# bharath5673/StrongSORT-YOLO

Measured on AMD Instinct MI355X. Metric: tracked frames/sec (whole node), 1280x720@30det, higher is better.
Workload: dtype f32 association / f64 Kalman+LSAP (f16 detector convs, fp32 ReID network on own v_mfma_f32 kernels)

## Files before the change

include/strongsort_hip.h:

```cpp
#ifndef STRONGSORT_HIP_H
#define STRONGSORT_HIP_H
#include <stdint.h>

#ifdef __cplusplus
extern "C" {
#endif

#define SS_OK 0
#define SS_ERR_INVALID (-1)
#define SS_ERR_CAPACITY (-2)
#define SS_ERR_HIP (-3)
#define SS_ERR_INFEASIBLE (-4)

#define SS_FEAT_DIM 512
#define SS_MAX_TRACKS 256
#define SS_MAX_DETS 128
#define SS_OUT_COLS 8

typedef struct ss_ctx ss_ctx;

typedef struct ss_config {
    double max_dist;
    double max_iou_distance;
    double mc_lambda;
// ... 165 lines not shown
                      void* d_out2, int c0, int cn);
int ss_op_bottleneck_f16(void* stream, const void* d_x, const void* d_w1, const void* d_b1, const void* d_w2, const void* d_b2,
                         int B, int H, int W, int C, int add, void* d_out, int out_ld, void* d_out2);
typedef struct ss_conv_desc {
    const void* x; const void* w; const void* bias; void* out;
    int B, H, W, Cin, N, ksize, stride, act;
} ss_conv_desc;
int ss_op_conv_group_f16(void* stream, int n, const ss_conv_desc* descs);
int ss_op_head_f16(void* stream, const void* d_x, const void* const* d_w1, const void* const* d_b1, const void* const* d_w2,
                   const void* const* d_b2, const void* const* d_w3, const void* const* d_b3, void* const* d_out, const int* nout,
                   int B, int H, int W, int Cin, int tile16);
int ss_op_v8_decode_f16(void* stream, const void* const* d_box, const void* const* d_cls, const void* const* d_box_bias,
                        const void* const* d_cls_bias, const int* H, const int* W, const int* strides, int B, int nc,
                        float* d_pred);
int ss_op_v8_decode_ext_f16(void* stream, const void* const* d_box, const void* const* d_cls, const void* const* d_box_bias,
                            const void* const* d_cls_bias, const void* const* d_ext, int n_ext, int ext_ld, int ext_mode,
                            const int* H, const int* W, const int* strides, int B, int nc, int cls_ld, float* d_pred);
int ss_op_dwconv3x3_f16(void* stream, const void* d_x, const void* d_w9 , const void* d_bias, void* d_y,
                        int N, int H, int W, int C, int act);
int ss_op_lightconv_f16(void* stream, const void* d_x, const void* d_w1, const void* d_w9, const void* d_bias,
                        void* d_y, int N, int H, int W, int C);
int ss_op_conv0_f16(void* stream, const void* d_x, const void* d_w_prep, const void* d_bias, void* d_y, int B, int H, int W, int Cout,
                    int act);
int ss_op_set_valid_images(void* stream, const int* d_n, int batch);
int ss_op_set_option(const char* name, int value);
int ss_op_osnet_stem_f16(void* stream, const void* d_x, const void* d_w_prep, const void* d_bias, void* d_y, int N, int H,
                         int W, const void* d_w1 , const void* d_b1, void* d_y1);
int ss_op_osnet_streams_bands(int N, int H, int W, int C);
int ss_op_osnet_streams_f16(void* stream, const void* d_x, const void* d_w1, const void* d_dwtab,
                            void* const* d_ys, float* d_psum, int N, int H, int W, int C);
long long ss_op_dwtab_bytes(int layers, int C);
int ss_op_dwtab_f16(void* stream, const void* d_w9, const void* d_bias, int layers, int C, void* d_out);
int ss_op_gate_apply_f16(void* stream, const void* const* d_xs, int T, const void* d_w1, const void* d_b1,
                         const void* d_w2, const void* d_b2, const float* d_sums, int parts, float scale, void* d_out,
                         int N, int HW, int C, int Cr);
int ss_op_osnet_tail_f16(void* stream, const void* const* d_ys, const float* d_psum, int parts, float scale, const void* d_gw1,
                         const void* d_gb1, const void* d_gw2, const void* d_gb2, int Cr, float* d_gates_ws ,
                         const void* d_w3, const void* d_b3, const void* d_idn, int C1, const void* d_wd, const void* d_bd,
                         void* d_out, const void* d_w4, const void* d_b4, void* d_out2, int pool, int N, int H, int W, int MID,
                         int C2, int N2);
int ss_op_upcat_f16(void* stream, const void* d_lo, const void* d_hi, void* d_out, int B, int h, int w, int C1, int C2, int lo_first);
int ss_op_sppf_pools_f16(void* stream, const void* d_x, void* d_out, int B, int H, int W, int C);
int ss_op_psa_attention_f16(void* stream, const void* d_qkv, const void* d_pe, void* d_out, int B, int N, int heads, float scale);
int ss_op_osnet_head_f16(void* stream, const void* d_x, const void* d_w, const void* d_bias, void* d_out, int N, int HW, int C, int F);
int ss_op_avgpool2_f16(void* stream, const void* d_x, void* d_y, int N, int H, int W, int C);
int ss_op_maxpool_f16(void* stream, const void* d_x, void* d_y, int N, int H, int W, int C, int k, int stride, int pad);
// ... 48 lines not shown
```

strongsort_yolo_amd/csrc/ss_front.hip:

```cpp
#include <hip/hip_fp16.h>
#include "ss_common.h"

__device__ inline void ss_axis(int d, float scale, int n_src, int& i0, int& i1, float& frac)
{
    float t = (float)d + 0.5f;
    float s = t * scale;
    float f = s - 0.5f;
    int i = (int)floorf(f);
    float fr = f - (float)i;
    if (i < 0) { i = 0; fr = 0.0f; }
    if (i >= n_src - 1) { i = n_src - 1; fr = 0.0f; i1 = i; } else i1 = i + 1;
    i0 = i; frac = fr;
}

__device__ inline float ss_bilerp_u8(float p00, float p01, float p10, float p11, float fx, float fy)
{
    float a = fmaf(fx, p01 - p00, p00);
    float b = fmaf(fx, p11 - p10, p10);
    float v = fmaf(fy, b - a, a);
    float q = floorf(v + 0.5f);
    return fminf(fmaxf(q, 0.0f), 255.0f);
}

template <typename T> __device__ inline T ss_cvt(float v);
template <> __device__ inline float ss_cvt<float>(float v) { return v; }
template <> __device__ inline __half ss_cvt<__half>(float v) { return __float2half(v); }
template <typename T> struct ss_is_u8 { static constexpr bool value = false; };
template <> struct ss_is_u8<uint8_t> { static constexpr bool value = true; };

template <typename T, int HWC>
__global__ __launch_bounds__(256) void k_letterbox(const uint8_t* __restrict__ src, long long src_batch_stride,
                                                   int H, int W, int stride, T* __restrict__ dst, int out_h,
                                                   int out_w, int new_h, int new_w, int pad_top, int pad_left,
                                                   float padv)
{
    const int x = blockIdx.x * blockDim.x + threadIdx.x;
    const int y = blockIdx.y;
    if (x >= out_w) return;
    const size_t plane = (size_t)out_h * out_w;
    src += (size_t)blockIdx.z * src_batch_stride;
    dst += (size_t)blockIdx.z * 3 * plane;
    const size_t o = HWC ? ((size_t)y * out_w + x) * 3 : (size_t)y * out_w + x;
    const size_t cs = HWC ? 1 : plane;
    const int ry = y - pad_top, rx = x - pad_left;
    if (ry < 0 || ry >= new_h || rx < 0 || rx >= new_w) {
        T p = ss_cvt<T>(padv);
        dst[o] = p; dst[cs + o] = p; dst[2 * cs + o] = p;
        return;
    }
    const float sx = (float)W / (float)new_w, sy = (float)H / (float)new_h;
    int y0, y1, x0, x1; float fy, fx;
    ss_axis(ry, sy, H, y0, y1, fy);
    ss_axis(rx, sx, W, x0, x1, fx);
    const uint8_t* r0 = src + (size_t)y0 * stride;
    const uint8_t* r1 = src + (size_t)y1 * stride;
#pragma unroll
    for (int c = 0; c < 3; ++c) {
        const int sc = 2 - c;
        float p00 = r0[x0 * 3 + sc], p01 = r0[x1 * 3 + sc], p10 = r1[x0 * 3 + sc], p11 = r1[x1 * 3 + sc];
        dst[c * cs + o] = ss_cvt<T>(ss_bilerp_u8(p00, p01, p10, p11, fx, fy) / 255.0f);
    }
}

void ss_launch_letterbox(const uint8_t* src, int batch, long long src_batch_stride, int h, int w, int stride, void* dst,
                         int flags, int out_h, int out_w, int new_h, int new_w, int pad_top, int pad_left,
                         int pad_value, hipStream_t st)
{
    if (batch <= 0) return;
    dim3 grid((out_w + 255) / 256, out_h, batch), block(256);
    float padv = (float)pad_value / 255.0f;
#define SS_LB(T, L) hipLaunchKernelGGL((k_letterbox<T, L>), grid, block, 0, st, src, src_batch_stride, h, w, stride, \
                                       (T*)dst, out_h, out_w, new_h, new_w, pad_top, pad_left, padv)
    switch (flags & 3) {
    case 0: SS_LB(float, 0); break;
    case 1: SS_LB(__half, 0); break;
    case 2: SS_LB(float, 1); break;
    default: SS_LB(__half, 1); break;
    }
#undef SS_LB
}

template <typename T, int HWC>
__global__ __launch_bounds__(128) void k_crop(const uint8_t* __restrict__ src, long long src_batch_stride, int H, int W,
// ... 714 lines not shown
```

strongsort_yolo_amd/csrc/ss_ops.hip:

```cpp
#include <hip/hip_fp16.h>
#include <hip/hip_runtime.h>
#include <stdint.h>
#include <stdlib.h>
#include <string>
#include "../../include/strongsort_hip.h"

struct NvEntry { void* stream; const int* n; int batch; };
static thread_local NvEntry g_nv[8] = {};
static inline const int* nv_for(void* stream, long long batch)
{
    for (const NvEntry& e : g_nv) if (e.n && e.stream == stream && e.batch == batch) return e.n;
    return nullptr;
}
static inline int nv_batch(void* stream)
{
    for (const NvEntry& e : g_nv) if (e.n && e.stream == stream) return e.batch;
    return 0;
}

static int g_opt_pw_epilogue = 1, g_opt_pw_splitk = 1, g_opt_osnet_chains = 1;

typedef _Float16 h8 __attribute__((ext_vector_type(8)));
typedef _Float16 h4 __attribute__((ext_vector_type(4)));
typedef float f4 __attribute__((ext_vector_type(4)));

__device__ inline float act_apply(float v, int act)
{
    if (act == 1) return v > 0.f ? v : 0.f;
// ... 941 lines not shown
        const h4 b1 = *reinterpret_cast<const h4*>(b1c + 4 * q);
#pragma unroll
        for (int pt = 0; pt < 2; ++pt) {
            const h8 bv = kv ? *reinterpret_cast<const h8*>(In + (size_t)(r * 32 + pt * 16 + n) * 24 + 8 * q) : z8;
            const h4 v0 = { bv[0], bv[1], bv[2], bv[3] }, v1 = { bv[4], bv[5], bv[6], bv[7] };
            f4 d = { 0.f, 0.f, 0.f, 0.f };
            d = __builtin_amdgcn_mfma_f32_16x16x16f16(a0, v0, d, 0, 0, 0);
            d = __builtin_amdgcn_mfma_f32_16x16x16f16(a1, v1, d, 0, 0, 0);
            h4 o;
#pragma unroll
            for (int j = 0; j < 4; ++j) {
                const float f = (float)(_Float16)d[j] + (float)b1[j];
                o[j] = (_Float16)(f > 0.f ? f : 0.f);
            }
            *reinterpret_cast<h4*>(y1 + (((size_t)img * OHp + j0 + r) * 32 + pt * 16 + n) * 16 + 4 * q) = o;
        }
    }
}

#define C0_PITCH 400
#define C0_ROWS 8

template <int COUT>
__global__ __launch_bounds__(256) void k_conv0(const __half* __restrict__ x, const __half* __restrict__ wp, const __half* __restrict__ bias,
                                              __half* __restrict__ y, int H, int W, int act)
{
    constexpr int MT = COUT / 16, IN_ROWS = 2 * C0_ROWS + 1, CH = C0_PITCH / 8;
    __shared__ __attribute__((aligned(16))) _Float16 In[IN_ROWS * C0_PITCH];
    const int tid = threadIdx.x, lane = tid & 63, r = tid >> 6, q = lane >> 4, n = lane & 15;
    const int OH = (H - 1) / 2 + 1, OW = W / 2;
    const int c0 = blockIdx.x * 64, oy0 = blockIdx.y * C0_ROWS, b = blockIdx.z;
    const h8 z8 = { 0, 0, 0, 0, 0, 0, 0, 0 };
    const __half* xi = x + (size_t)b * H * W * 3;
    const int row_halfs = W * 3, f0 = 6 * c0 - 8;
    for (int i = tid; i < IN_ROWS * CH; i += 256) {
        const int rr = i / CH, ch = i - rr * CH, gr = 2 * oy0 - 1 + rr, f = f0 + ch * 8;
        *reinterpret_cast<h8*>(In + rr * C0_PITCH + ch * 8) =
            (gr >= 0 && gr < H && f >= 0 && f + 8 <= row_halfs) ? *reinterpret_cast<const h8*>(xi + (size_t)gr * row_halfs + f) : z8;
    }
    h4 a[MT][3], bb[MT];
#pragma unroll
    for (int mt = 0; mt < MT; ++mt) {
#pragma unroll
        for (int ky = 0; ky < 3; ++ky) a[mt][ky] = *reinterpret_cast<const h4*>(wp + ((size_t)(r * 3 + ky) * COUT + mt * 16 + n) * 16 + 4 * q);
        bb[mt] = *reinterpret_cast<const h4*>(bias + mt * 16 + 4 * q);
    }
    __syncthreads();
    const _Float16* bp = In + 8 * (3 * n + (6 * r + 5) / 8) + 4 * q;
    const int c = c0 + 4 * n + r;
#pragma unroll 2
    for (int cr = 0; cr < C0_ROWS; ++cr) {
        const int oy = oy0 + cr;
        if (oy >= OH) break;
        h4 bv[3];
#pragma unroll
        for (int ky = 0; ky < 3; ++ky) bv[ky] = *reinterpret_cast<const h4*>(bp + (2 * cr + ky) * C0_PITCH);
#pragma unroll
        for (int mt = 0; mt < MT; ++mt) {
            f4 d = { 0.f, 0.f, 0.f, 0.f };
#pragma unroll
            for (int ky = 0; ky < 3; ++ky) d = __builtin_amdgcn_mfma_f32_16x16x16f16(a[mt][ky], bv[ky], d, 0, 0, 0);
            h4 o;
#pragma unroll
            for (int j = 0; j < 4; ++j) o[j] = (_Float16)act_apply((float)(_Float16)d[j] + (float)bb[mt][j], act);
            if (c < OW) *reinterpret_cast<h4*>(y + (((size_t)b * OH + oy) * OW + c) * COUT + mt * 16 + 4 * q) = o;
        }
    }
}

#define LC_TH 16

template <int C>
struct DwDiag {
    static constexpr int MT = (C + 15) / 16;
    h8 A1[MT][3], A2[MT][3];
    f4 bf[MT];
    __device__ __forceinline__ void init(const __half* __restrict__ w9l, const __half* __restrict__ biasl, int q, int n)
    {
#pragma unroll
        for (int mt = 0; mt < MT; ++mt) {
            const int c = mt * 16 + n, c4 = mt * 16 + 4 * q;
            const bool on = c < C && (n >> 2) == q;
#pragma unroll
            for (int ky = 0; ky < 3; ++ky) {
                const _Float16 w0 = on ? (_Float16)__half2float(w9l[(ky * 3 + 0) * C + c]) : (_Float16)0.f;
                const _Float16 w1 = on ? (_Float16)__half2float(w9l[(ky * 3 + 1) * C + c]) : (_Float16)0.f;
                const _Float16 w2 = on ? (_Float16)__half2float(w9l[(ky * 3 + 2) * C + c]) : (_Float16)0.f;
                h8 a1 = { 0, 0, 0, 0, 0, 0, 0, 0 }, a2 = { 0, 0, 0, 0, 0, 0, 0, 0 };
#pragma unroll
                for (int j = 0; j < 4; ++j) {
// ... 1535 lines not shown

extern "C" int ss_op_sppf_pools_f16(void* stream, const void* x, void* out, int B, int H, int W, int C)
{
    if (!x || !out || B < 1 || H < 1 || W < 1 || C < 8 || C % 8 || H * W > 1024) return SS_ERR_INVALID;
    hipLaunchKernelGGL(k_sppf_pools, dim3((unsigned)(B * (C / 8))), dim3(256), (size_t)2 * H * W * 16, (hipStream_t)stream,
                       (const __half*)x, (__half*)out, H, W, C / 8);
    return hipGetLastError() == hipSuccess ? SS_OK : SS_ERR_HIP;
}

extern "C" int ss_op_conv0_f16(void* stream, const void* x, const void* w_prep, const void* bias, void* y, int B, int H, int W, int Cout,
                               int act)
{
    if (!x || !w_prep || !bias || !y || B < 1 || H < 2 || W < 128 || W % 128 || (W * 3) % 8 || (Cout != 16 && Cout != 32 && Cout != 48))
        return SS_ERR_INVALID;
    const int OH = (H - 1) / 2 + 1;
    const dim3 grid(W / 128, (OH + C0_ROWS - 1) / C0_ROWS, B), block(256);
    hipStream_t st = (hipStream_t)stream;
#define SS_C0(CO) hipLaunchKernelGGL(k_conv0<CO>, grid, block, 0, st, (const __half*)x, (const __half*)w_prep, (const __half*)bias, (__half*)y, H, W, act)
    if (Cout == 16) SS_C0(16); else if (Cout == 32) SS_C0(32); else SS_C0(48);
#undef SS_C0
    return hipGetLastError() == hipSuccess ? SS_OK : SS_ERR_HIP;
}

extern "C" int ss_op_bottleneck_f16(void* stream, const void* x, const void* w1, const void* b1, const void* w2, const void* b2, int B, int H,
                                    int W, int C, int add, void* out, int out_ld, void* out2)
{
    if (!x || !w1 || !b1 || !w2 || !b2 || !out || B < 1 || H < 1 || W < 1 || (C != 16 && C != 32 && C != 64 && C != 128) || out_ld < C || out_ld % 4 ||
        ((uintptr_t)out % 8) || ((uintptr_t)x % 16) || ((uintptr_t)w1 % 16) || ((uintptr_t)w2 % 16) || (out2 && ((uintptr_t)out2 % 8)))
        return SS_ERR_INVALID;
    const long long M = (long long)B * H * W;
    const bool big = M / 128 >= 512 && C <= 64;
    BnArgs A{ (const __half*)x, (const __half*)w1, (const __half*)b1, (const __half*)w2, (const __half*)b2, (__half*)out, out_ld, (__half*)out2,
              B, H, W, add, big ? 16 : 8, 8, 0, 0 };
    A.tiles_x = (W + A.TW - 1) / A.TW; A.tiles_y = (H + A.TH - 1) / A.TH;
    const int P = C + 8;
    const size_t lds = ((size_t)(A.TH + 4) * (A.TW + 4) * P + (((size_t)(A.TH + 2) * (A.TW + 2) * P + 7) & ~(size_t)7) + 2 * (size_t)C * 72) * 2 + 128;
    const dim3 grid((unsigned)(B * A.tiles_x * A.tiles_y));
    hipStream_t st = (hipStream_t)stream;
#define SS_BN(CC, P1, P2) do { static unsigned long long attr = 0; int dv_ = 0; (void)hipGetDevice(&dv_); if (!(attr >> (dv_ & 63) & 1)) { (void)hipFuncSetAttribute((const void*)k_bneck<CC, P1, P2>, hipFuncAttributeMaxDynamicSharedMemorySize, 160 * 1024 - 512); attr |= 1ull << (dv_ & 63); }    \
                               hipLaunchKernelGGL((k_bneck<CC, P1, P2>), grid, dim3(256), lds, st, A); } while (0)
    if (big) { if (C == 16) SS_BN(16, 3, 2); else if (C == 32) SS_BN(32, 3, 2); else SS_BN(64, 3, 2); }
    else { if (C == 16) SS_BN(16, 2, 1); else if (C == 32) SS_BN(32, 2, 1); else if (C == 64) SS_BN(64, 2, 1); else SS_BN(128, 2, 1); }
#undef SS_BN
    return hipGetLastError() == hipSuccess ? SS_OK : SS_ERR_HIP;
}

// ... 58 lines not shown
```

strongsort_yolo_amd/fused.py:

```python
from __future__ import annotations

import ctypes as C
import threading

import torch

from . import lib as _lib

import os as _os

ENABLED = True


def _flag(name: str) -> bool:
    return True


FLAG_NAMES = ("POINTWISE", "CONV3X3", "BNECK", "GROUP", "HEAD", "HEAD_TILE16", "LIGHTCONV", "CONV0", "STEM", "STEM_CONV1", "STREAMS", "TAIL", "GLUE", "DW3X3", "HEAD_EXT", "C3K2", "PSA", "OSHEAD")


def set_flags(**kw):
    g, old = globals(), {}
    for k, v in kw.items():
        if k not in FLAG_NAMES and k != "BNECK_C":
            raise ValueError(f"unknown fused switch {k!r}")
        old[k] = g[k]
        g[k] = tuple(int(c) for c in v) if k == "BNECK_C" else bool(v)
    return old


def flags_from_env(env=None):
    env = _os.environ if env is None else env
    kw = {n: env["SS_FUSED_" + n] != "0" for n in FLAG_NAMES if "SS_FUSED_" + n in env}
    if "SS_BNECK_C" in env:
        kw["BNECK_C"] = tuple(int(c) for c in env["SS_BNECK_C"].split(","))
    return set_flags(**kw)

ACT = {"none": 0, "relu": 1, "silu": 2, "sigmoid": 3}


def usable(x: torch.Tensor) -> bool:
# ... 373 lines not shown
    n, c, h, w = x.shape
    return (CONV0 and usable(x) and c == 3 and w % 128 == 0 and h >= 2 and conv.kernel_size == (3, 3) and conv.stride == (2, 2)
            and conv.padding == (1, 1) and conv.dilation == (1, 1) and conv.groups == 1 and conv.out_channels in (16, 32, 48)
            and conv.bias is not None)


def conv0_weight(mod, conv):
    def build():
        co = conv.out_channels
        taps = conv.weight.detach().permute(2, 0, 3, 1).reshape(3, co, 9)
        w = torch.zeros(4, 3, co, 16, dtype=conv.weight.dtype, device=conv.weight.device)
        for r in range(4):
            sh = (6 * r + 5) % 8
            w[r, :, :, sh:sh + 9] = taps
        return w
    return _cached(mod, "_w_c0", conv.weight, build)


def conv0(x, w_prep, bias, act="silu"):
    x = _cl(x)
    n, c, h, w = x.shape
    co = w_prep.shape[2]
    y = new_cl(x, co, ((h - 1) // 2 + 1, w // 2))
    _ck(_lib.load().ss_op_conv0_f16(_st(x), _p(x), _p(w_prep), _p(bias), _p(y), n, h, w, co, ACT[act]))
    return y


STEM = _flag("STEM")


def stem_ok(x, conv) -> bool:
    n, c, h, w = x.shape
    return (STEM and c == 3 and w == 128 and h % 16 == 0 and conv.kernel_size == (7, 7) and conv.stride == (2, 2)
            and conv.padding == (3, 3) and conv.out_channels == 16 and conv.groups == 1 and conv.bias is not None)


def stem_weight(mod, conv):
    def build():
        taps = conv.weight.detach().permute(2, 0, 3, 1).reshape(7, 16, 21)
        w = torch.zeros(4, 7, 16, 32, dtype=conv.weight.dtype, device=conv.weight.device)
        for r in range(4):
            sh = (6 * r + 7) % 8
            w[r, :, :, sh:sh + 21] = taps
        return w
    return _cached(mod, "_w_stem", conv.weight, build)


STEM_CONV1 = _flag("STEM_CONV1")
# ... 187 lines not shown
```

strongsort_yolo_amd/lib.py:

```python
from __future__ import annotations

import ctypes as C
import os
import subprocess

_HERE = os.path.dirname(os.path.abspath(__file__))
SO_PATH = os.environ.get("SS_LIB_PATH") or os.path.join(_HERE, "libstrongsort_hip.so")
CSRC = os.path.join(_HERE, "csrc")

SS_OK, SS_ERR_INVALID, SS_ERR_CAPACITY, SS_ERR_HIP, SS_ERR_INFEASIBLE = 0, -1, -2, -3, -4
MAX_TRACKS, MAX_DETS, FEAT_DIM, OUT_COLS = 256, 128, 512, 8
DST_F16, DST_HWC, DST_U8 = 1, 2, 4

EXPORTS = [
    "ss_create", "ss_destroy", "ss_last_error", "ss_set_hip_stream", "ss_reset", "ss_synchronize",
    "ss_upload", "ss_upload_batch", "ss_download", "ss_overlay_set_font", "ss_overlay", "ss_letterbox", "ss_letterbox_batch", "ss_nms", "ss_nms_batch", "ss_nms_set_classes", "ss_crop_norm", "ss_crop_norm_batch",
    "ss_track_update", "ss_track_update_group", "ss_cmc_estimate", "ss_track_set_cmc", "ss_crop_norm_packed", "ss_unpack_feats", "ss_pack_results", "ss_op_set_valid_images", "ss_op_set_option", "ss_track_set_assoc_event", "ss_track_update_host",
    "ss_check_errors", "ss_set_option", "ss_feat_normalize", "ss_ema", "ss_kf_predict", "ss_kf_update", "ss_kf_project", "ss_kf_initiate",
    "ss_gallery_pack", "ss_assoc_cost", "ss_iou_cost", "ss_lsap", "ss_get_tracks", "ss_get_debug",
    "ss_get_gallery", "ss_max_group_frames", "ss_track_join", "ss_stream_create", "ss_stream_destroy", "ss_assoc_timing", "ss_assoc_timing_values", "ss_assoc_inkernel_timing", "ss_assoc_timeline", "ss_op_bias_act_f16", "ss_op_bias_act_place_f16", "ss_op_pointwise_f16", "ss_op_conv3x3_f16", "ss_op_bottleneck_f16", "ss_op_conv_group_f16", "ss_op_head_f16", "ss_op_v8_decode_f16", "ss_op_v8_decode_ext_f16", "ss_op_dwconv3x3_f16", "ss_op_lightconv_f16", "ss_op_osnet_stem_f16", "ss_op_conv0_f16", "ss_op_osnet_streams_f16", "ss_op_osnet_streams_bands", "ss_op_dwtab_bytes", "ss_op_dwtab_f16", "ss_op_gate_apply_f16", "ss_op_osnet_tail_f16", "ss_op_gate_sum_f16", "ss_op_avgpool2_f16", "ss_op_upcat_f16", "ss_op_sppf_pools_f16", "ss_op_psa_attention_f16", "ss_op_osnet_head_f16", "ss_op_maxpool_f16",
    "ss_op32_pointwise", "ss_op32_chains_bands", "ss_op32_chains", "ss_op32_tail", "ss_op32_stem", "ss_op32_stem_u8", "ss_op32_stem_conv1", "ss_op32_head", "ss_op32_set_option", "ss_op32_conv", "ss_op32_conv0", "ss_op32_upcat", "ss_op32_v8_decode", "ss_op32_sppf_pools",
    "ss_mask_assemble", "ss_mask_outline",
    "ss_byte_create", "ss_byte_destroy", "ss_byte_update_group", "ss_byte_update", "ss_byte_reset", "ss_byte_get_tracks",
    "ss_byte_set_gmc", "ss_byte_set_reid", "ss_byte_update_group_feats", "ss_byte_get_features",
    "ss_native_feats",
    "ss_byte_set_pose", "ss_byte_update_group_kpts", "ss_byte_get_keypoints", "ss_byte_get_det_keypoints",
    "ss_gmc_sparse_estimate", "ss_gmc_sparse_get",
    "ss_jpeg_probe", "ss_jpeg_coefficients", "ss_jpeg_decode_batch",
    "ss_jpeg_encode_bound", "ss_jpeg_entropy_encode", "ss_jpeg_encode_batch",
]


class SSError(RuntimeError):
    def __init__(self, code, msg):
        super().__init__(f"strongsort_hip error {code}: {msg}")
        self.code = code


class ss_config(C.Structure):
    _fields_ = [
        ("max_dist", C.c_double), ("max_iou_distance", C.c_double), ("mc_lambda", C.c_double),
        ("gating_threshold", C.c_double), ("gated_cost", C.c_double),
        ("std_weight_position", C.c_double), ("std_weight_velocity", C.c_double),
# ... 90 lines not shown
    L.ss_iou_cost.argtypes = [vp, dp, i, dp, i, dp]
    L.ss_lsap.argtypes = [vp, dp, i, i, ip]
    hd, hu8 = C.POINTER(C.c_double), C.POINTER(C.c_uint8)
    L.ss_get_tracks.argtypes = [vp, i, i, hi, hi, hi, hi, hi, hi, hi, hi, hf, hd, hd, hf, hi]
    L.ss_get_debug.argtypes = [vp, i, i, hi, hf, hd, hu8, hd, hd, hi]
    L.ss_get_gallery.argtypes = [vp, i, i, hf, i, hi]
    L.ss_assoc_timing.argtypes = [vp, i, hf, hi]
    L.ss_assoc_timing_values.argtypes = [vp, hf, i, hi]
    L.ss_assoc_inkernel_timing.argtypes = [vp, i, C.POINTER(C.c_double), hi]
    L.ss_assoc_timeline.argtypes = [vp, C.POINTER(C.c_longlong), i]
    L.ss_op_bias_act_f16.argtypes = [vp, vp, vp, vp, C.c_longlong, i, i]
    L.ss_op_dwconv3x3_f16.argtypes = [vp, vp, vp, vp, vp, i, i, i, i, i]
    L.ss_op_bias_act_place_f16.argtypes = [vp, vp, vp, vp, C.c_longlong, i, i, i, vp, i, vp, i, i]
    L.ss_op_pointwise_f16.argtypes = [vp, vp, vp, vp, vp, C.c_longlong, i, i, i, i, vp, i, vp, i, i]
    L.ss_op_conv3x3_f16.argtypes = [vp, vp, vp, vp, vp, i, i, i, i, i, i, i, i, vp, i, vp, i, i]
    L.ss_op_bottleneck_f16.argtypes = [vp, vp, vp, vp, vp, vp, i, i, i, i, i, vp, i, vp]
    L.ss_op_conv_group_f16.argtypes = [vp, i, C.POINTER(ss_conv_desc)]
    pv = C.POINTER(vp)
    L.ss_op_head_f16.argtypes = [vp, vp, pv, pv, pv, pv, pv, pv, pv, C.POINTER(C.c_int), i, i, i, i, i]
    L.ss_op_v8_decode_f16.argtypes = [vp, C.POINTER(vp), C.POINTER(vp), C.POINTER(vp), C.POINTER(vp), hi, hi, hi, i, i, vp]
    L.ss_op_v8_decode_ext_f16.argtypes = [vp, C.POINTER(vp), C.POINTER(vp), C.POINTER(vp), C.POINTER(vp), C.POINTER(vp), i, i, i, hi, hi, hi, i, i, i, vp]
    L.ss_op_lightconv_f16.argtypes = [vp, vp, vp, vp, vp, vp, i, i, i, i]
    L.ss_op_conv0_f16.argtypes = [vp, vp, vp, vp, vp, i, i, i, i, i]
    L.ss_op_osnet_stem_f16.argtypes = [vp, vp, vp, vp, vp, i, i, i, vp, vp, vp]
    L.ss_op_osnet_streams_f16.argtypes = [vp, vp, vp, vp, C.POINTER(vp), vp, i, i, i, i]
    L.ss_op_dwtab_bytes.argtypes = [i, i]
    L.ss_op_dwtab_bytes.restype = C.c_longlong
    L.ss_op_dwtab_f16.argtypes = [vp, vp, vp, i, i, vp]
    L.ss_op_osnet_streams_bands.argtypes = [i, i, i, i]
    L.ss_op_gate_apply_f16.argtypes = [vp, C.POINTER(vp), i, vp, vp, vp, vp, vp, i, f, vp, i, i, i, i]
    L.ss_op_osnet_tail_f16.argtypes = [vp, C.POINTER(vp), vp, i, f, vp, vp, vp, vp, i, vp, vp, vp, vp, i, vp, vp, vp, vp, vp, vp, i, i, i, i, i, i, i]
    L.ss_op_upcat_f16.argtypes = [vp, vp, vp, vp, i, i, i, i, i, i]
    L.ss_op_sppf_pools_f16.argtypes = [vp, vp, vp, i, i, i, i]
    L.ss_op_psa_attention_f16.argtypes = [vp, vp, vp, vp, i, i, i, C.c_float]
    L.ss_op_osnet_head_f16.argtypes = [vp, vp, vp, vp, vp, i, i, i, i]
    L.ss_op_avgpool2_f16.argtypes = [vp, vp, vp, i, i, i, i]
    L.ss_op_maxpool_f16.argtypes = [vp, vp, vp, i, i, i, i, i, i, i]
    L.ss_op_gate_sum_f16.argtypes = [vp, C.POINTER(vp), i, vp, vp, vp, vp, vp, vp, i, i, i, i]
    L.ss_op32_pointwise.argtypes = [vp, vp, vp, vp, vp, vp, ll, i, i, i, vp, i]
    L.ss_op32_chains_bands.argtypes = [i, i, i, i]
    L.ss_op32_chains.argtypes = [vp, vp, vp, vp, vp, C.POINTER(vp), vp, i, i, i, i, vp]
    L.ss_op32_tail.argtypes = [vp, C.POINTER(vp), vp, i, vp, vp, vp, vp, i, vp, vp, vp, vp, i, vp, vp, vp, vp, vp, vp, i, i, i, i, i, i, i, vp]
    L.ss_op32_stem.argtypes = [vp, vp, vp, vp, vp, i, i, i, vp]
    L.ss_op32_stem_u8.argtypes = [vp, vp, vp, vp, vp, i, i, i, vp]
    L.ss_op32_stem_conv1.argtypes = [vp, vp, i, vp, vp, vp, vp, vp, vp, i, i, i, vp]
    L.ss_op32_head.argtypes = [vp, vp, vp, vp, vp, i, i, i, i, vp]
# ... 57 lines not shown
```

strongsort_yolo_amd/pipeline.py:

```python
from __future__ import annotations

from typing import Optional

import numpy as np
import torch

from .config import StrongSortConfig, DetectConfig
from .engine import TrackerEngine, letterbox_geometry, scale_geometry
from .lib import MAX_DETS, MAX_TRACKS, FEAT_DIM
from . import nets


class FramePipeline:
    def __init__(self, detector: str = "yolov8n", n_streams: int = 1, frame_hw=(720, 1280), device: int = 0,
                 half: bool = True, reid_batch: int = 32, cfg: Optional[StrongSortConfig] = None,
                 dcfg: Optional[DetectConfig] = None, det_source: str = "detector", feat_source: str = "reid",
                 graph: str = "all", debug: bool = False, run_nets: bool = True, seed: int = 0, detect_only_rows: int = 0, cmc: bool = False,
                 reid_half: Optional[bool] = None, crops_u8: bool = True, tracker: str = "strongsort", with_reid: bool = False,
                 reid_model: str = "osnet", with_pose: bool = False, gmc_method: str = "ecc"):
        self.cfg, self.dcfg = cfg or StrongSortConfig(), dcfg or DetectConfig()
        self.S, (self.H, self.W) = n_streams, frame_hw
        from .config import byte_config, check_reid_model, check_pose, check_gmc_method
        self.byte_cfg = byte_config(tracker, with_reid, with_pose)
        self.gmc_method = check_gmc_method(gmc_method, cmc, tracker)
# ... 46 lines not shown
        self.n_anchors = sum((g.out_h // s) * (g.out_w // s) for s in (8, 16, 32))
        self.F, self.Sv, self.pack, self.keep_net_outputs = 1, S, False, False
        self.cmc = bool(cmc)
        b = self.b = _Bufs(self, S, self.det_rows, 1, self.cmc)
        for name in ("frames", "lb", "pred_in", "dets", "dets6", "proto", "keep", "ndets", "crops", "anchor_gt", "gt_feats", "warps"):
            setattr(self, name, getattr(b, name))
        self.feats_in = b.feats_v
        self.geom_dev = torch.tensor([[self.gain, self.pad_x, self.pad_y, float(self.W), float(self.H)]] * S,
                                     dtype=torch.float32, device=dev)
        self.img_hw = torch.tensor([[self.H, self.W]] * S, dtype=torch.int32, device=dev)
        self.out, self.nout = self.eng.out, self.eng.nout
        self._maps = None
        self.graph = None
        self.graph_all = None
        self.graph_mode = graph
        if self.cmc:
            self.eng.estimate_warps(self.gmc_method, self.frames, 1, self.warps)
            self.reset_tracker(-1)
            self.trk.set_cmc(self.warps)

    grouped = False

    def _letterbox(self, b):
        if self.cmc:
            self.eng.estimate_warps(self.gmc_method, b.frames, self.F, b.warps, n_valid=b.nvalid)
        if self.run_nets:
            self.eng.letterbox_batch(b.frames, self.geom, half=self.half, pad_value=self.dcfg.pad_value, out=b.lb,
                                     channels_last=True)

    @staticmethod
    def _keep(b, name, tensors):
        cur = getattr(b, name, None)
        if cur is None:
            cur = [torch.empty_like(t) for t in tensors]
            setattr(b, name, cur)
        for d, t in zip(cur, tensors):
            d.copy_(t)

    def _s_backbone(self, b):
        if self.run_nets:
            self._letterbox(b)
            self._keep(b, "pyr", self.detector.forward_backbone(b.lb))

    def _s_head(self, b):
        self._forward(b, lambda: self.detector.forward_head(*b.pyr))

    def _s_detector(self, b):
        if self.run_nets:
            self._letterbox(b)
            self._forward(b, lambda: self.detector(b.lb))
        elif self.cmc and not self.grouped:
            self._letterbox(b)

    def _forward(self, b, head):
        with self._decode_into(b.pred_in):
            pred = self._pred(head(), b.proto)
        if self.native:
            b.maps, self._maps = self._maps, None
        if self.keep_net_outputs:
            b.head_out = pred
        if self.det_source == "detector" and pred.data_ptr() != b.pred_in.data_ptr():
            b.pred_in.copy_(pred)

    def _nms(self, b):
        e = self.eng
        e.nms_batch(b.pred_in, self.nc, self.dcfg, self.geom_dev, n_extra=self.nx, rows=b.dets, keep=b.keep,
                    count=b.ndets, max_det=self.max_det)
        if self.nx:
            b.dets6.copy_(b.dets[:, :, :6])
        if self.native and self.run_nets and self.feat_source == "reid":
            e.native_feats(b.maps, b.keep, b.ndets, b.feats_v)
        if not self.grouped:
            b.maps = None
# ... 424 lines not shown
```

Measured before the change: 8528.

## Fuse letterbox resize into the first detector convolution

New measurement: 8629, median of 4. 1.2% higher.

```diff
diff --git a/include/strongsort_hip.h b/include/strongsort_hip.h
--- a/include/strongsort_hip.h
+++ b/include/strongsort_hip.h
@@ -211,6 +211,9 @@
                         void* d_y, int N, int H, int W, int C);
 int ss_op_conv0_f16(void* stream, const void* d_x, const void* d_w_prep, const void* d_bias, void* d_y, int B, int H, int W, int Cout,
                     int act);
+int ss_op_conv0_letterbox_f16(void* stream, const uint8_t* d_src, int batch, long long src_batch_stride, int h, int w, int stride,
+                              int out_h, int out_w, int new_h, int new_w, int pad_top, int pad_left, int pad_value,
+                              const void* d_w_prep, const void* d_bias, void* d_y, int Cout, int act, void* d_lb);
 int ss_op_set_valid_images(void* stream, const int* d_n, int batch);
 int ss_op_set_option(const char* name, int value);
 int ss_op_osnet_stem_f16(void* stream, const void* d_x, const void* d_w_prep, const void* d_bias, void* d_y, int N, int H,
diff --git a/strongsort_yolo_amd/csrc/ss_front.hip b/strongsort_yolo_amd/csrc/ss_front.hip
--- a/strongsort_yolo_amd/csrc/ss_front.hip
+++ b/strongsort_yolo_amd/csrc/ss_front.hip
@@ -1,26 +1,6 @@
 #include <hip/hip_fp16.h>
 #include "ss_common.h"
-
-__device__ inline void ss_axis(int d, float scale, int n_src, int& i0, int& i1, float& frac)
-{
-    float t = (float)d + 0.5f;
-    float s = t * scale;
-    float f = s - 0.5f;
-    int i = (int)floorf(f);
-    float fr = f - (float)i;
-    if (i < 0) { i = 0; fr = 0.0f; }
-    if (i >= n_src - 1) { i = n_src - 1; fr = 0.0f; i1 = i; } else i1 = i + 1;
-    i0 = i; frac = fr;
-}
-
-__device__ inline float ss_bilerp_u8(float p00, float p01, float p10, float p11, float fx, float fy)
-{
-    float a = fmaf(fx, p01 - p00, p00);
-    float b = fmaf(fx, p11 - p10, p10);
-    float v = fmaf(fy, b - a, a);
-    float q = floorf(v + 0.5f);
-    return fminf(fmaxf(q, 0.0f), 255.0f);
-}
+#include "ss_resample.h"
 
 template <typename T> __device__ inline T ss_cvt(float v);
 template <> __device__ inline float ss_cvt<float>(float v) { return v; }
@@ -58,7 +38,7 @@
     for (int c = 0; c < 3; ++c) {
         const int sc = 2 - c;
         float p00 = r0[x0 * 3 + sc], p01 = r0[x1 * 3 + sc], p10 = r1[x0 * 3 + sc], p11 = r1[x1 * 3 + sc];
-        dst[c * cs + o] = ss_cvt<T>(ss_bilerp_u8(p00, p01, p10, p11, fx, fy) / 255.0f);
+        dst[c * cs + o] = ss_cvt<T>(ss_unit255(ss_bilerp_u8(p00, p01, p10, p11, fx, fy)));
     }
 }
 
diff --git a/strongsort_yolo_amd/csrc/ss_ops.hip b/strongsort_yolo_amd/csrc/ss_ops.hip
--- a/strongsort_yolo_amd/csrc/ss_ops.hip
+++ b/strongsort_yolo_amd/csrc/ss_ops.hip
@@ -4,6 +4,7 @@
 #include <stdlib.h>
 #include <string>
 #include "../../include/strongsort_hip.h"
+#include "ss_resample.h"
 
 struct NvEntry { void* stream; const int* n; int batch; };
 static thread_local NvEntry g_nv[8] = {};
@@ -991,12 +992,48 @@
 #define C0_ROWS 8
 
 template <int COUT>
+__device__ __forceinline__ void conv0_tile(const _Float16* In, const __half* __restrict__ wp, const __half* __restrict__ bias, __half* __restrict__ y,
+                                           int OH, int OW, int c0, int oy0, int b, int act)
+{
+    constexpr int MT = COUT / 16;
+    const int tid = threadIdx.x, lane = tid & 63, r = tid >> 6, q = lane >> 4, n = lane & 15;
+    h4 a[MT][3], bb[MT];
+#pragma unroll
+    for (int mt = 0; mt < MT; ++mt) {
+#pragma unroll
+        for (int ky = 0; ky < 3; ++ky) a[mt][ky] = *reinterpret_cast<const h4*>(wp + ((size_t)(r * 3 + ky) * COUT + mt * 16 + n) * 16 + 4 * q);
+        bb[mt] = *reinterpret_cast<const h4*>(bias + mt * 16 + 4 * q);
+    }
+    __syncthreads();
+    const _Float16* bp = In + 8 * (3 * n + (6 * r + 5) / 8) + 4 * q;
+    const int c = c0 + 4 * n + r;
+#pragma unroll 2
+    for (int cr = 0; cr < C0_ROWS; ++cr) {
+        const int oy = oy0 + cr;
+        if (oy >= OH) break;
+        h4 bv[3];
+#pragma unroll
+        for (int ky = 0; ky < 3; ++ky) bv[ky] = *reinterpret_cast<const h4*>(bp + (2 * cr + ky) * C0_PITCH);
+#pragma unroll
+        for (int mt = 0; mt < MT; ++mt) {
+            f4 d = { 0.f, 0.f, 0.f, 0.f };
+#pragma unroll
+            for (int ky = 0; ky < 3; ++ky) d = __builtin_amdgcn_mfma_f32_16x16x16f16(a[mt][ky], bv[ky], d, 0, 0, 0);
+            h4 o;
+#pragma unroll
+            for (int j = 0; j < 4; ++j) o[j] = (_Float16)act_apply((float)(_Float16)d[j] + (float)bb[mt][j], act);
+            if (c < OW) *reinterpret_cast<h4*>(y + (((size_t)b * OH + oy) * OW + c) * COUT + mt * 16 + 4 * q) = o;
+        }
+    }
+}
+
+template <int COUT>
 __global__ __launch_bounds__(256) void k_conv0(const __half* __restrict__ x, const __half* __restrict__ wp, const __half* __restrict__ bias,
                                               __half* __restrict__ y, int H, int W, int act)
 {
-    constexpr int MT = COUT / 16, IN_ROWS = 2 * C0_ROWS + 1, CH = C0_PITCH / 8;
+    constexpr int IN_ROWS = 2 * C0_ROWS + 1, CH = C0_PITCH / 8;
     __shared__ __attribute__((aligned(16))) _Float16 In[IN_ROWS * C0_PITCH];
-    const int tid = threadIdx.x, lane = tid & 63, r = tid >> 6, q = lane >> 4, n = lane & 15;
+    const int tid = threadIdx.x;
     const int OH = (H - 1) / 2 + 1, OW = W / 2;
     const int c0 = blockIdx.x * 64, oy0 = blockIdx.y * C0_ROWS, b = blockIdx.z;
     const h8 z8 = { 0, 0, 0, 0, 0, 0, 0, 0 };
@@ -1007,34 +1044,102 @@
         *reinterpret_cast<h8*>(In + rr * C0_PITCH + ch * 8) =
             (gr >= 0 && gr < H && f >= 0 && f + 8 <= row_halfs) ? *reinterpret_cast<const h8*>(xi + (size_t)gr * row_halfs + f) : z8;
     }
-    h4 a[MT][3], bb[MT];
-#pragma unroll
-    for (int mt = 0; mt < MT; ++mt) {
-#pragma unroll
-        for (int ky = 0; ky < 3; ++ky) a[mt][ky] = *reinterpret_cast<const h4*>(wp + ((size_t)(r * 3 + ky) * COUT + mt * 16 + n) * 16 + 4 * q);
-        bb[mt] = *reinterpret_cast<const h4*>(bias + mt * 16 + 4 * q);
+    conv0_tile<COUT>(In, wp, bias, y, OH, OW, c0, oy0, b, act);
+}
+
+struct C0Frame {
+    const uint8_t* src; long long batch_stride;
+    int H, W, stride, new_h, new_w, pad_top, pad_left;
+    float padv;
+};
+#define C0_COLS 136
+#define C0_ZERO (-1)
+#define C0_PAD (-2)
+
+template <int COUT>
+__global__ __launch_bounds__(256) void k_conv0_lb(C0Frame g, const __half* __restrict__ wp, const __half* __restrict__ bias, __half* __restrict__ y,
+                                                 __half* __restrict__ lb, int H, int W, int act)
+{
+    constexpr int IN_ROWS = 2 * C0_ROWS + 1, CH = C0_PITCH / 8;
+    __shared__ __attribute__((aligned(16))) _Float16 In[IN_ROWS * C0_PITCH];
+    __shared__ unsigned short lut[256];
+    __shared__ int cs[C0_COLS], csh[C0_COLS], ry0[IN_ROWS], ry1[IN_ROWS];
+    __shared__ float cfx[C0_COLS], rfy[IN_ROWS];
+    const int tid = threadIdx.x;
+    const int OH = (H - 1) / 2 + 1, OW = W / 2;
+    const int c0 = blockIdx.x * 64, oy0 = blockIdx.y * C0_ROWS, b = blockIdx.z;
+    const uint8_t* src = g.src + (size_t)b * g.batch_stride;
+    lut[tid] = __half_as_ushort(__float2half(ss_unit255((float)tid)));
+    if (tid < C0_COLS) {
+        const int x = 2 * c0 - 3 + tid, rx = x - g.pad_left;
+        int s = C0_ZERO, sh = 0; float fx = 0.f;
+        if (x >= 0 && x < W) {
+            s = C0_PAD;
+            if (rx >= 0 && rx < g.new_w) {
+                int x0, x1;
+                ss_axis(rx, (float)g.W / (float)g.new_w, g.W, x0, x1, fx);
+                s = max(3 * x1 - 5, 0);
+                sh = (8 * (3 * x0 - s)) | ((8 * (3 * x1 - s)) << 8);
+            }
+        }
+        cs[tid] = s; csh[tid] = sh; cfx[tid] = fx;
+    } else if (tid >= 192 && tid < 192 + IN_ROWS) {
+        const int rr = tid - 192, gr = 2 * oy0 - 1 + rr, ry = gr - g.pad_top;
+        int y0 = C0_ZERO, y1 = 0; float fy = 0.f;
+        if (gr >= 0 && gr < H) {
+            y0 = C0_PAD;
+            if (ry >= 0 && ry < g.new_h) ss_axis(ry, (float)g.H / (float)g.new_h, g.H, y0, y1, fy);
+        }
+        ry0[rr] = y0; ry1[rr] = y1; rfy[rr] = fy;
     }
     __syncthreads();
-    const _Float16* bp = In + 8 * (3 * n + (6 * r + 5) / 8) + 4 * q;
-    const int c = c0 + 4 * n + r;
-#pragma unroll 2
-    for (int cr = 0; cr < C0_ROWS; ++cr) {
-        const int oy = oy0 + cr;
-        if (oy >= OH) break;
-        h4 bv[3];
-#pragma unroll
-        for (int ky = 0; ky < 3; ++ky) bv[ky] = *reinterpret_cast<const h4*>(bp + (2 * cr + ky) * C0_PITCH);
-#pragma unroll
-        for (int mt = 0; mt < MT; ++mt) {
-            f4 d = { 0.f, 0.f, 0.f, 0.f };
-#pragma unroll
-            for (int ky = 0; ky < 3; ++ky) d = __builtin_amdgcn_mfma_f32_16x16x16f16(a[mt][ky], bv[ky], d, 0, 0, 0);
-            h4 o;
-#pragma unroll
-            for (int j = 0; j < 4; ++j) o[j] = (_Float16)act_apply((float)(_Float16)d[j] + (float)bb[mt][j], act);
-            if (c < OW) *reinterpret_cast<h4*>(y + (((size_t)b * OH + oy) * OW + c) * COUT + mt * 16 + 4 * q) = o;
-        }
-    }
+    const unsigned padh = __half_as_ushort(__float2half(g.padv));
+    __half* lbi = lb ? lb + (size_t)b * H * W * 3 : nullptr;
+    const int row_halfs = W * 3, f0 = 6 * c0 - 8;
+    for (int i = tid; i < IN_ROWS * CH; i += 256) {
+        const int rr = i / CH, ch = i - rr * CH, t = 1 + 8 * ch, i0 = t / 3, ph = t - 3 * i0;
+        const int y0 = ry0[rr], y1 = ry1[rr];
+        const float fy = rfy[rr];
+        const bool rs = y0 >= 0;
+        const uint8_t* r0 = src + (size_t)(rs ? y0 : 0) * g.stride;
+        const uint8_t* r1 = src + (size_t)(rs ? y1 : 0) * g.stride;
+        int s[4], sh[4]; float fx[4];
+        unsigned long long ta[4], tb[4];
+#pragma unroll
+        for (int j = 0; j < 4; ++j) {
+            const bool used = j < 3 || ph == 2;
+            s[j] = used ? cs[i0 + j] : C0_ZERO; sh[j] = used ? csh[i0 + j] : 0; fx[j] = used ? cfx[i0 + j] : 0.f;
+            ta[j] = tb[j] = 0;
+            if (rs && s[j] >= 0) { __builtin_memcpy(&ta[j], r0 + s[j], 8); __builtin_memcpy(&tb[j], r1 + s[j], 8); }
+        }
+        unsigned v[12];
+#pragma unroll
+        for (int j = 0; j < 4; ++j) {
+            const unsigned a0 = (unsigned)(ta[j] >> (sh[j] & 255)), a1 = (unsigned)(ta[j] >> (sh[j] >> 8));
+            const unsigned b0 = (unsigned)(tb[j] >> (sh[j] & 255)), b1 = (unsigned)(tb[j] >> (sh[j] >> 8));
+            const unsigned other = (y0 == C0_ZERO || s[j] == C0_ZERO) ? 0u : padh;
+#pragma unroll
+            for (int c = 0; c < 3; ++c) {
+                const int bs = 8 * (2 - c);
+                const float p00 = (float)((a0 >> bs) & 255u), p01 = (float)((a1 >> bs) & 255u), p10 = (float)((b0 >> bs) & 255u),
+                            p11 = (float)((b1 >> bs) & 255u);
+                const unsigned smp = lut[(int)ss_bilerp_u8(p00, p01, p10, p11, fx[j], fy)];
+                v[3 * j + c] = (rs && s[j] >= 0) ? smp : other;
+            }
+        }
+        uint4 o;
+        unsigned* ow = reinterpret_cast<unsigned*>(&o);
+#pragma unroll
+        for (int k = 0; k < 4; ++k) {
+            const unsigned lo = ph == 0 ? v[2 * k] : ph == 1 ? v[2 * k + 1] : v[2 * k + 2];
+            const unsigned hi = ph == 0 ? v[2 * k + 1] : ph == 1 ? v[2 * k + 2] : v[2 * k + 3];
+            ow[k] = lo | (hi << 16);
+        }
+        *reinterpret_cast<uint4*>(In + rr * C0_PITCH + ch * 8) = o;
+        const int gr = 2 * oy0 - 1 + rr;
+        if (lbi && rr >= 1 && ch >= 1 && ch <= CH - 2 && gr < H) *reinterpret_cast<uint4*>(lbi + (size_t)gr * row_halfs + f0 + ch * 8) = o;
+    }
+    conv0_tile<COUT>(In, wp, bias, y, OH, OW, c0, oy0, b, act);
 }
 
 #define LC_TH 16
@@ -2616,6 +2721,24 @@
     return hipGetLastError() == hipSuccess ? SS_OK : SS_ERR_HIP;
 }
 
+extern "C" int ss_op_conv0_letterbox_f16(void* stream, const uint8_t* src, int batch, long long src_batch_stride, int h, int w, int stride,
+                                         int out_h, int out_w, int new_h, int new_w, int pad_top, int pad_left, int pad_value,
+                                         const void* w_prep, const void* bias, void* y, int Cout, int act, void* lb)
+{
+    if (!src || !w_prep || !bias || !y || batch < 1 || batch > 65535 || h < 1 || w < 3 || stride < 3 * w || src_batch_stride < 0 || out_h < 2 ||
+        out_w < 128 || out_w % 128 || new_h < 1 || new_w < 1 || (Cout != 16 && Cout != 32 && Cout != 48) || ((uintptr_t)lb % 16) || ((uintptr_t)y % 8))
+        return SS_ERR_INVALID;
+    const int OH = (out_h - 1) / 2 + 1;
+    if ((OH + C0_ROWS - 1) / C0_ROWS > 65535) return SS_ERR_INVALID;
+    const dim3 grid(out_w / 128, (OH + C0_ROWS - 1) / C0_ROWS, batch), block(256);
+    const C0Frame g{ src, src_batch_stride, h, w, stride, new_h, new_w, pad_top, pad_left, (float)pad_value / 255.0f };
+    hipStream_t st = (hipStream_t)stream;
+#define SS_C0(CO) hipLaunchKernelGGL(k_conv0_lb<CO>, grid, block, 0, st, g, (const __half*)w_prep, (const __half*)bias, (__half*)y, (__half*)lb, out_h, out_w, act)
+    if (Cout == 16) SS_C0(16); else if (Cout == 32) SS_C0(32); else SS_C0(48);
+#undef SS_C0
+    return hipGetLastError() == hipSuccess ? SS_OK : SS_ERR_HIP;
+}
+
 extern "C" int ss_op_bottleneck_f16(void* stream, const void* x, const void* w1, const void* b1, const void* w2, const void* b2, int B, int H,
                                     int W, int C, int add, void* out, int out_ld, void* out2)
 {
diff --git a/strongsort_yolo_amd/csrc/ss_resample.h b/strongsort_yolo_amd/csrc/ss_resample.h
--- /dev/null
+++ b/strongsort_yolo_amd/csrc/ss_resample.h
@@ -0,0 +1,25 @@
+#pragma once
+#include <hip/hip_runtime.h>
+
+__device__ inline void ss_axis(int d, float scale, int n_src, int& i0, int& i1, float& frac)
+{
+    float t = (float)d + 0.5f;
+    float s = t * scale;
+    float f = s - 0.5f;
+    int i = (int)floorf(f);
+    float fr = f - (float)i;
+    if (i < 0) { i = 0; fr = 0.0f; }
+    if (i >= n_src - 1) { i = n_src - 1; fr = 0.0f; i1 = i; } else i1 = i + 1;
+    i0 = i; frac = fr;
+}
+
+__device__ inline float ss_bilerp_u8(float p00, float p01, float p10, float p11, float fx, float fy)
+{
+    float a = fmaf(fx, p01 - p00, p00);
+    float b = fmaf(fx, p11 - p10, p10);
+    float v = fmaf(fy, b - a, a);
+    float q = floorf(v + 0.5f);
+    return fminf(fmaxf(q, 0.0f), 255.0f);
+}
+
+__device__ inline float ss_unit255(float q) { return q / 255.0f; }
diff --git a/strongsort_yolo_amd/fused.py b/strongsort_yolo_amd/fused.py
--- a/strongsort_yolo_amd/fused.py
+++ b/strongsort_yolo_amd/fused.py
@@ -16,7 +16,7 @@
     return True
 
 
-FLAG_NAMES = ("POINTWISE", "CONV3X3", "BNECK", "GROUP", "HEAD", "HEAD_TILE16", "LIGHTCONV", "CONV0", "STEM", "STEM_CONV1", "STREAMS", "TAIL", "GLUE", "DW3X3", "HEAD_EXT", "C3K2", "PSA", "OSHEAD")
+FLAG_NAMES = ("POINTWISE", "CONV3X3", "BNECK", "GROUP", "HEAD", "HEAD_TILE16", "LIGHTCONV", "CONV0", "CONV0_LB", "STEM", "STEM_CONV1", "STREAMS", "TAIL", "GLUE", "DW3X3", "HEAD_EXT", "C3K2", "PSA", "OSHEAD")
 
 
 def set_flags(**kw):
@@ -436,8 +436,50 @@
     n, c, h, w = x.shape
     co = w_prep.shape[2]
     y = new_cl(x, co, ((h - 1) // 2 + 1, w // 2))
+    src = conv0_frames.take(x)
+    if src is not None:
+        f, g = src.frames, src.geom
+        _ck(_lib.load().ss_op_conv0_letterbox_f16(_st(x), _p(f), f.shape[0], f.stride(0), f.shape[1], f.shape[2], f.stride(1), g.out_h, g.out_w,
+                                                  g.new_h, g.new_w, g.pad_top, g.pad_left, src.pad_value, _p(w_prep), _p(bias), _p(y), co, ACT[act], _p(x)))
+        return y
     _ck(_lib.load().ss_op_conv0_f16(_st(x), _p(x), _p(w_prep), _p(bias), _p(y), n, h, w, co, ACT[act]))
     return y
+
+
+CONV0_LB = _flag("CONV0_LB")
+
+
+class conv0_frames:
+    _tls = threading.local()
+
+    def __init__(self, frames, geom, pad_value, lb):
+        self.frames, self.geom, self.pad_value, self.lb = frames, geom, int(pad_value), lb
+
+    @staticmethod
+    def ok(frames, geom, lb, conv) -> bool:
+        return (CONV0_LB and conv0_ok(lb, conv) and lb.is_contiguous(memory_format=torch.channels_last) and frames.is_cuda
+                and frames.dtype == torch.uint8 and frames.dim() == 4 and frames.shape[0] == lb.shape[0] and frames.shape[2] >= 3
+                and frames.shape[3] == 3 and frames.stride(3) == 1 and frames.stride(2) == 3
+                and tuple(lb.shape[2:]) == (geom.out_h, geom.out_w))
+
+    def __enter__(self):
+        self.prev = getattr(conv0_frames._tls, "cur", None)
+        conv0_frames._tls.cur = self
+        return self
+
+    def __exit__(self, *exc):
+        pending, conv0_frames._tls.cur = conv0_frames._tls.cur is self, self.prev
+        if pending and exc[0] is None:
+            raise RuntimeError("conv0_frames: no first convolution read the letterbox buffer")
+        return False
+
+    @staticmethod
+    def take(x):
+        cur = getattr(conv0_frames._tls, "cur", None)
+        if cur is None or x.data_ptr() != cur.lb.data_ptr() or x.shape != cur.lb.shape:
+            return None
+        conv0_frames._tls.cur = None
+        return cur
 
 
 STEM = _flag("STEM")
diff --git a/strongsort_yolo_amd/lib.py b/strongsort_yolo_amd/lib.py
--- a/strongsort_yolo_amd/lib.py
+++ b/strongsort_yolo_amd/lib.py
@@ -18,7 +18,7 @@
     "ss_track_update", "ss_track_update_group", "ss_cmc_estimate", "ss_track_set_cmc", "ss_crop_norm_packed", "ss_unpack_feats", "ss_pack_results", "ss_op_set_valid_images", "ss_op_set_option", "ss_track_set_assoc_event", "ss_track_update_host",
     "ss_check_errors", "ss_set_option", "ss_feat_normalize", "ss_ema", "ss_kf_predict", "ss_kf_update", "ss_kf_project", "ss_kf_initiate",
     "ss_gallery_pack", "ss_assoc_cost", "ss_iou_cost", "ss_lsap", "ss_get_tracks", "ss_get_debug",
-    "ss_get_gallery", "ss_max_group_frames", "ss_track_join", "ss_stream_create", "ss_stream_destroy", "ss_assoc_timing", "ss_assoc_timing_values", "ss_assoc_inkernel_timing", "ss_assoc_timeline", "ss_op_bias_act_f16", "ss_op_bias_act_place_f16", "ss_op_pointwise_f16", "ss_op_conv3x3_f16", "ss_op_bottleneck_f16", "ss_op_conv_group_f16", "ss_op_head_f16", "ss_op_v8_decode_f16", "ss_op_v8_decode_ext_f16", "ss_op_dwconv3x3_f16", "ss_op_lightconv_f16", "ss_op_osnet_stem_f16", "ss_op_conv0_f16", "ss_op_osnet_streams_f16", "ss_op_osnet_streams_bands", "ss_op_dwtab_bytes", "ss_op_dwtab_f16", "ss_op_gate_apply_f16", "ss_op_osnet_tail_f16", "ss_op_gate_sum_f16", "ss_op_avgpool2_f16", "ss_op_upcat_f16", "ss_op_sppf_pools_f16", "ss_op_psa_attention_f16", "ss_op_osnet_head_f16", "ss_op_maxpool_f16",
+    "ss_get_gallery", "ss_max_group_frames", "ss_track_join", "ss_stream_create", "ss_stream_destroy", "ss_assoc_timing", "ss_assoc_timing_values", "ss_assoc_inkernel_timing", "ss_assoc_timeline", "ss_op_bias_act_f16", "ss_op_bias_act_place_f16", "ss_op_pointwise_f16", "ss_op_conv3x3_f16", "ss_op_bottleneck_f16", "ss_op_conv_group_f16", "ss_op_head_f16", "ss_op_v8_decode_f16", "ss_op_v8_decode_ext_f16", "ss_op_dwconv3x3_f16", "ss_op_lightconv_f16", "ss_op_osnet_stem_f16", "ss_op_conv0_f16", "ss_op_conv0_letterbox_f16", "ss_op_osnet_streams_f16", "ss_op_osnet_streams_bands", "ss_op_dwtab_bytes", "ss_op_dwtab_f16", "ss_op_gate_apply_f16", "ss_op_osnet_tail_f16", "ss_op_gate_sum_f16", "ss_op_avgpool2_f16", "ss_op_upcat_f16", "ss_op_sppf_pools_f16", "ss_op_psa_attention_f16", "ss_op_osnet_head_f16", "ss_op_maxpool_f16",
     "ss_op32_pointwise", "ss_op32_chains_bands", "ss_op32_chains", "ss_op32_tail", "ss_op32_stem", "ss_op32_stem_u8", "ss_op32_stem_conv1", "ss_op32_head", "ss_op32_set_option", "ss_op32_conv", "ss_op32_conv0", "ss_op32_upcat", "ss_op32_v8_decode", "ss_op32_sppf_pools",
     "ss_mask_assemble", "ss_mask_outline",
     "ss_byte_create", "ss_byte_destroy", "ss_byte_update_group", "ss_byte_update", "ss_byte_reset", "ss_byte_get_tracks",
@@ -155,6 +155,7 @@
     L.ss_op_v8_decode_ext_f16.argtypes = [vp, C.POINTER(vp), C.POINTER(vp), C.POINTER(vp), C.POINTER(vp), C.POINTER(vp), i, i, i, hi, hi, hi, i, i, i, vp]
     L.ss_op_lightconv_f16.argtypes = [vp, vp, vp, vp, vp, vp, i, i, i, i]
     L.ss_op_conv0_f16.argtypes = [vp, vp, vp, vp, vp, i, i, i, i, i]
+    L.ss_op_conv0_letterbox_f16.argtypes = [vp, vp, i, C.c_longlong, i, i, i, i, i, i, i, i, i, i, vp, vp, vp, i, i, vp]
     L.ss_op_osnet_stem_f16.argtypes = [vp, vp, vp, vp, vp, i, i, i, vp, vp, vp]
     L.ss_op_osnet_streams_f16.argtypes = [vp, vp, vp, vp, C.POINTER(vp), vp, i, i, i, i]
     L.ss_op_dwtab_bytes.argtypes = [i, i]
diff --git a/strongsort_yolo_amd/pipeline.py b/strongsort_yolo_amd/pipeline.py
--- a/strongsort_yolo_amd/pipeline.py
+++ b/strongsort_yolo_amd/pipeline.py
@@ -92,11 +92,17 @@
     grouped = False
 
     def _letterbox(self, b):
+        import contextlib
+        from . import fused
         if self.cmc:
             self.eng.estimate_warps(self.gmc_method, b.frames, self.F, b.warps, n_valid=b.nvalid)
         if self.run_nets:
+            b0 = getattr(self.detector, "b0", None)
+            if isinstance(b0, nets.Conv) and b0.conv.in_channels == 3 and fused.conv0_frames.ok(b.frames, self.geom, b.lb, b0.conv):
+                return fused.conv0_frames(b.frames, self.geom, self.dcfg.pad_value, b.lb)
             self.eng.letterbox_batch(b.frames, self.geom, half=self.half, pad_value=self.dcfg.pad_value, out=b.lb,
                                      channels_last=True)
+        return contextlib.nullcontext()
 
     @staticmethod
     def _keep(b, name, tensors):
@@ -109,16 +115,16 @@
 
     def _s_backbone(self, b):
         if self.run_nets:
-            self._letterbox(b)
-            self._keep(b, "pyr", self.detector.forward_backbone(b.lb))
+            with self._letterbox(b):
+                self._keep(b, "pyr", self.detector.forward_backbone(b.lb))
 
     def _s_head(self, b):
         self._forward(b, lambda: self.detector.forward_head(*b.pyr))
 
     def _s_detector(self, b):
         if self.run_nets:
-            self._letterbox(b)
-            self._forward(b, lambda: self.detector(b.lb))
+            with self._letterbox(b):
+                self._forward(b, lambda: self.detector(b.lb))
         elif self.cmc and not self.grouped:
             self._letterbox(b)
 
```
